# zju3dv/ENeRF

Hardware: AMD Instinct MI355X
Metric: rendered frames/sec @512x640 3-src-view (higher is better)
Workload: dtype f32

## Files before the change

### enerf_amd/csrc/common.h

```cpp
#pragma once

#ifdef ENERF_EMU
#include "hip_emu.h"
typedef emu_f32x4 f32x4;
#else
#include <hip/hip_runtime.h>
typedef float f32x4 __attribute__((ext_vector_type(4)));
#define ENERF_LAUNCH(kern, grid, block, shmem, stream, ...) \
    hipLaunchKernelGGL(kern, dim3(grid), dim3(block), (shmem), (stream), __VA_ARGS__)
#define ENERF_LAUNCH_SIMPLE ENERF_LAUNCH
#define ENERF_DYN_SMEM(type, name) \
    extern __shared__ __attribute__((aligned(16))) char enerf_dyn_smem_[]; \
    type* name = reinterpret_cast<type*>(enerf_dyn_smem_)
#define ENERF_OPAQUE_V(x) asm volatile("" : "+v"(x))
#endif
#ifdef ENERF_EMU
#define ENERF_OPAQUE_V(x) (void)(x)
#endif

#include <stdint.h>

namespace enerf {

__device__ __forceinline__ void wave_sync() {
// ... 170 lines not shown
}
__device__ __forceinline__ float group_max4(float v) {
#ifdef ENERF_EMU
    v = fmaxf(v, __shfl_xor(v, 16));
    v = fmaxf(v, __shfl_xor(v, 32));
    return v;
#else
    unsigned u = __float_as_uint(v);
    auto r = __builtin_amdgcn_permlane32_swap(u, u, false, false);
    v = fmaxf(__uint_as_float(r[0]), __uint_as_float(r[1]));
    u = __float_as_uint(v);
    r = __builtin_amdgcn_permlane16_swap(u, u, false, false);
    return fmaxf(__uint_as_float(r[0]), __uint_as_float(r[1]));
#endif
}

__device__ __forceinline__ unsigned xcd_contiguous(unsigned bid, unsigned nblk) {
    const unsigned q = nblk / 8, r = nblk % 8, xcd = bid % 8, k = bid / 8;
    return (xcd < r ? xcd * (q + 1) : r * (q + 1) + (xcd - r) * q) + k;
}
__host__ __device__ __forceinline__ long long cdivl(long long a, long long b) { return (a + b - 1) / b; }

struct Lerp1 {
    int i0, i1;
    float l0, l1;
};
__host__ __device__ __forceinline__ float ac_scale(int in, int out) {
    return out > 1 ? (float)(in - 1) / (float)(out - 1) : 0.f;
}
__host__ __device__ __forceinline__ Lerp1 ac_lerp(int dst, float scale, int in) {
    Lerp1 r;
    float src = scale * (float)dst;
    r.i0 = (int)src;
    if (r.i0 > in - 1) r.i0 = in - 1;
    r.i1 = r.i0 + (r.i0 < in - 1 ? 1 : 0);
    r.l1 = src - (float)r.i0;
    r.l0 = 1.f - r.l1;
    return r;
}
__host__ __device__ __forceinline__ float ac_blend(const Lerp1& y, const Lerp1& x, float v00, float v01, float v10,
                                                   float v11) {
    return y.l0 * (x.l0 * v00 + x.l1 * v01) + y.l1 * (x.l0 * v10 + x.l1 * v11);
}

__host__ __device__ __forceinline__ float gs_unnorm(float g, int size) { return ((g + 1.f) * 0.5f) * (float)(size - 1); }

struct Taps2 {
    int x0, x1, y0, y1;
    float w00, w01, w10, w11;
};
__device__ __forceinline__ int mul24(int a, int b) {
#ifdef ENERF_EMU
    return a * b;
#else
    return __mul24(a, b);
#endif
}

template <bool BORDER>
__host__ __device__ __forceinline__ Taps2 gs_taps2(float ix, float iy, int W, int H) {
    Taps2 t;
    if (BORDER) {
        ix = fminf((float)(W - 1), fmaxf(ix, 0.f));
        iy = fminf((float)(H - 1), fmaxf(iy, 0.f));
        const float fx = floorf(ix), fy = floorf(iy);
        t.x0 = (int)fx; t.y0 = (int)fy;
        t.x1 = t.x0 + 1 < W ? t.x0 + 1 : W - 1;
        t.y1 = t.y0 + 1 < H ? t.y0 + 1 : H - 1;
        const float tx1 = ix - fx, ty1 = iy - fy, tx0 = (fx + 1.f) - ix, ty0 = (fy + 1.f) - iy;
        t.w00 = tx0 * ty0; t.w01 = tx1 * ty0; t.w10 = tx0 * ty1; t.w11 = tx1 * ty1;
        return t;
    }
    bool finite = (ix > -1e8f) && (ix < 1e8f) && (iy > -1e8f) && (iy < 1e8f);
    if (!finite) { ix = -10.f; iy = -10.f; }
    float fx = floorf(ix), fy = floorf(iy);
    int x0 = (int)fx, y0 = (int)fy;
    int x1 = x0 + 1, y1 = y0 + 1;
    float tx1 = ix - fx, ty1 = iy - fy;
    float tx0 = (float)x1 - ix, ty0 = (float)y1 - iy;
    bool vx0 = x0 >= 0 && x0 < W, vx1 = x1 >= 0 && x1 < W;
    bool vy0 = y0 >= 0 && y0 < H, vy1 = y1 >= 0 && y1 < H;
    t.w00 = (vx0 && vy0) ? tx0 * ty0 : 0.f;
    t.w01 = (vx1 && vy0) ? tx1 * ty0 : 0.f;
    t.w10 = (vx0 && vy1) ? tx0 * ty1 : 0.f;
    t.w11 = (vx1 && vy1) ? tx1 * ty1 : 0.f;
    t.x0 = x0 < 0 ? 0 : (x0 > W - 1 ? W - 1 : x0);
    t.x1 = x1 < 0 ? 0 : (x1 > W - 1 ? W - 1 : x1);
    t.y0 = y0 < 0 ? 0 : (y0 > H - 1 ? H - 1 : y0);
    t.y1 = y1 < 0 ? 0 : (y1 > H - 1 ? H - 1 : y1);
    return t;
}

__device__ __forceinline__ float clamp_min(float v, float lo) { return v < lo ? lo : v; }

__device__ __forceinline__ void atomic_add_f32(float* p, float v) {
#ifdef ENERF_EMU
    atomicAdd(p, v);
#else
    unsafeAtomicAdd(p, v);
#endif
}

__device__ __forceinline__ void lds_add_f32(float* p, float v) {
#ifdef ENERF_EMU
    atomicAdd(p, v);
#else
    __builtin_amdgcn_ds_faddf((__attribute__((address_space(3))) float*)p, v, 0, 0, false);
#endif
}

#ifdef ENERF_EMU
__device__ __forceinline__ float fast_rcp(float x) { return 1.f / x; }
__device__ __forceinline__ float fast_sqrt(float x) { return sqrtf(x); }
__device__ __forceinline__ float fast_exp(float x) { return expf(x); }
#else
__device__ __forceinline__ float fast_rcp(float x) { return __builtin_amdgcn_rcpf(x); }
__device__ __forceinline__ float fast_sqrt(float x) { return __builtin_amdgcn_sqrtf(x); }
__device__ __forceinline__ float fast_exp(float x) { return __expf(x); }
#endif

__host__ __device__ __forceinline__ float linspace01(int k, int D) {
    if (D == 1) return 0.f;
    float step = 1.f / (float)(D - 1);
    return k < D / 2 ? step * (float)k : 1.f - step * (float)(D - 1 - k);
}

__host__ __device__ __forceinline__ bool inv4x4(const double* m, double* inv) {
    inv[0] = m[5] * m[10] * m[15] - m[5] * m[11] * m[14] - m[9] * m[6] * m[15] + m[9] * m[7] * m[14] + m[13] * m[6] * m[11] - m[13] * m[7] * m[10];
    inv[4] = -m[4] * m[10] * m[15] + m[4] * m[11] * m[14] + m[8] * m[6] * m[15] - m[8] * m[7] * m[14] - m[12] * m[6] * m[11] + m[12] * m[7] * m[10];
    inv[8] = m[4] * m[9] * m[15] - m[4] * m[11] * m[13] - m[8] * m[5] * m[15] + m[8] * m[7] * m[13] + m[12] * m[5] * m[11] - m[12] * m[7] * m[9];
    inv[12] = -m[4] * m[9] * m[14] + m[4] * m[10] * m[13] + m[8] * m[5] * m[14] - m[8] * m[6] * m[13] - m[12] * m[5] * m[10] + m[12] * m[6] * m[9];
    inv[1] = -m[1] * m[10] * m[15] + m[1] * m[11] * m[14] + m[9] * m[2] * m[15] - m[9] * m[3] * m[14] - m[13] * m[2] * m[11] + m[13] * m[3] * m[10];
    inv[5] = m[0] * m[10] * m[15] - m[0] * m[11] * m[14] - m[8] * m[2] * m[15] + m[8] * m[3] * m[14] + m[12] * m[2] * m[11] - m[12] * m[3] * m[10];
    inv[9] = -m[0] * m[9] * m[15] + m[0] * m[11] * m[13] + m[8] * m[1] * m[15] - m[8] * m[3] * m[13] - m[12] * m[1] * m[11] + m[12] * m[3] * m[9];
    inv[13] = m[0] * m[9] * m[14] - m[0] * m[10] * m[13] - m[8] * m[1] * m[14] + m[8] * m[2] * m[13] + m[12] * m[1] * m[10] - m[12] * m[2] * m[9];
    inv[2] = m[1] * m[6] * m[15] - m[1] * m[7] * m[14] - m[5] * m[2] * m[15] + m[5] * m[3] * m[14] + m[13] * m[2] * m[7] - m[13] * m[3] * m[6];
    inv[6] = -m[0] * m[6] * m[15] + m[0] * m[7] * m[14] + m[4] * m[2] * m[15] - m[4] * m[3] * m[14] - m[12] * m[2] * m[7] + m[12] * m[3] * m[6];
    inv[10] = m[0] * m[5] * m[15] - m[0] * m[7] * m[13] - m[4] * m[1] * m[15] + m[4] * m[3] * m[13] + m[12] * m[1] * m[7] - m[12] * m[3] * m[5];
    inv[14] = -m[0] * m[5] * m[14] + m[0] * m[6] * m[13] + m[4] * m[1] * m[14] - m[4] * m[2] * m[13] - m[12] * m[1] * m[6] + m[12] * m[2] * m[5];
    inv[3] = -m[1] * m[6] * m[11] + m[1] * m[7] * m[10] + m[5] * m[2] * m[11] - m[5] * m[3] * m[10] - m[9] * m[2] * m[7] + m[9] * m[3] * m[6];
    inv[7] = m[0] * m[6] * m[11] - m[0] * m[7] * m[10] - m[4] * m[2] * m[11] + m[4] * m[3] * m[10] + m[8] * m[2] * m[7] - m[8] * m[3] * m[6];
    inv[11] = -m[0] * m[5] * m[11] + m[0] * m[7] * m[9] + m[4] * m[1] * m[11] - m[4] * m[3] * m[9] - m[8] * m[1] * m[7] + m[8] * m[3] * m[5];
    inv[15] = m[0] * m[5] * m[10] - m[0] * m[6] * m[9] - m[4] * m[1] * m[10] + m[4] * m[2] * m[9] + m[8] * m[1] * m[6] - m[8] * m[2] * m[5];
    double det = m[0] * inv[0] + m[1] * inv[4] + m[2] * inv[8] + m[3] * inv[12];
    if (det == 0.0) return false;
    double r = 1.0 / det;
    for (int i = 0; i < 16; ++i) inv[i] *= r;
    return true;
}

struct RayBounds {
    float rn, rf, vn, vf;
};
__device__ __forceinline__ RayBounds ray_bounds(float ru, float rv, const float* __restrict__ pd,
                                                const float* __restrict__ ps, const float* __restrict__ n0,
                                                int h, int w, int Hr, int Wr, int depth_inv) {
    int u = (int)ru, v = (int)rv;
    u = u < 0 ? u + Wr : u;
    v = v < 0 ? v + Hr : v;
    u = u < 0 ? 0 : (u > Wr - 1 ? Wr - 1 : u);
    v = v < 0 ? 0 : (v > Hr - 1 ? Hr - 1 : v);
    const Lerp1 ly = ac_lerp(v, ac_scale(h, Hr), h), lx = ac_lerp(u, ac_scale(w, Wr), w);
    const int o00 = ly.i0 * w + lx.i0, o01 = ly.i0 * w + lx.i1, o10 = ly.i1 * w + lx.i0, o11 = ly.i1 * w + lx.i1;
    const float* n1 = n0 + h * w;
    float d, s, a0, a1;
    if ((h == Hr) && (w == Wr)) {
        d = pd[o00]; s = ps[o00]; a0 = n0[o00]; a1 = n1[o00];
    } else {
        d = ac_blend(ly, lx, pd[o00], pd[o01], pd[o10], pd[o11]);
        s = ac_blend(ly, lx, ps[o00], ps[o01], ps[o10], ps[o11]);
        a0 = ac_blend(ly, lx, n0[o00], n0[o01], n0[o10], n0[o11]);
        a1 = ac_blend(ly, lx, n1[o00], n1[o01], n1[o10], n1[o11]);
    }
    RayBounds r;
    if (depth_inv) {
        r.rn = d + s; if (r.rn > a0) r.rn = a0;
        r.rf = d - s; if (r.rf < a1) r.rf = a1;
    } else {
        r.rn = d - s; if (r.rn < a0) r.rn = a0;
        r.rf = d + s; if (r.rf > a1) r.rf = a1;
    }
    r.vn = a0; r.vf = a1;
    return r;
}

}
```

### enerf_amd/csrc/render.hip

```cpp
#include "nerf_layout.h"

#ifndef ENERF_RENDER_PREFETCH
#define ENERF_RENDER_PREFETCH 0
#endif

namespace enerf {

__host__ __device__ __forceinline__ int bx_image_floats(int F, int pieces = 3) { return F == 11 ? bx_layout().tiles * 256 * pieces : 0; }
long long nerf_packed_floats(int F) { return nerf_layout(F).total + bx_image_floats(F); }

__host__ __device__ __forceinline__ int slot_channel(int g, int r, int R, int F) {
    int c = g * R + r;
    return (r < R && c < F) ? c : -1;
}

__device__ __forceinline__ float bx_weight(const NerfRaw& w, int F, int e, int g, int j, int q) {
    const int R = (F + 3) / 4, CI = 88 + F + 4;
    const BxLayout B = bx_layout();
    const int half = q >> 2, r = q & 3;
    const int c = (r < R && g * R + r < F) ? g * R + r : -1;
    if (e < B.ga) return c >= 0 ? w.glob_w[(16 * e + j) * 3 * F + (1 + half) * F + c] : 0.f;
    if (e < B.fc) return (half == 0 && c >= 0) ? w.glob_w[(16 * (e - B.ga) + j) * 3 * F + c] : 0.f;
    if (e < B.lr0) return w.fc_w[j * 32 + 16 * half + 4 * g + r];
    if (e < B.c0p) {
        const int unit = 16 * (e - B.lr0) + j;
        if (half == 0) return r < 2 ? w.lr0_w[unit * 24 + 2 * g + r] : 0.f;
        return w.lr0_w[unit * 24 + 8 + 4 * g + r];
    }
    if (e < B.c0v) {
        const int pr = (e - B.c0p) >> 2, unit = 16 * ((e - B.c0p) & 3) + j;
        if (pr < 2) return w.col0_w[unit * CI + 16 * (2 * pr + half) + 4 * g + r];
        if (half == 0) return r < 2 ? w.col0_w[unit * CI + 64 + 2 * g + r] : 0.f;
        return w.col0_w[unit * CI + 72 + 4 * g + r];
    }
    if (half) return 0.f;
    const int unit = 16 * (e - B.c0v) + j;
    if (c >= 0) return w.col0_w[unit * CI + 88 + c];
    return r == R ? w.col0_w[unit * CI + 88 + F + g] : 0.f;
}
__device__ __forceinline__ unsigned bf16_bits_rne(float f) {
    unsigned u = __float_as_uint(f);
    return (u + 0x7fffu + ((u >> 16) & 1u)) >> 16;
}
__global__ __launch_bounds__(256) void k_nerf_pack(NerfRaw w, int F, int viewdir_agg, float* __restrict__ out) {
    const NerfLayout L = nerf_layout(F);
    int i = blockIdx.x * blockDim.x + threadIdx.x;
    if (i >= L.total + bx_image_floats(F)) return;
    if (i >= L.total) {
        const int idx = i - L.total, n_plane = bx_layout().tiles * 256;
        const int piece = idx / n_plane, k = idx - piece * n_plane;
        const int e = k >> 8, lane = (k >> 2) & 63, wq = k & 3;
        unsigned word = 0;
        for (int h = 0; h < 2; ++h) {
            float rem = bx_weight(w, F, e, lane >> 4, lane & 15, 2 * wq + h);
            unsigned bits = 0;
            for (int pc = 0; pc <= piece; ++pc) { bits = bf16_bits_rne(rem); rem -= __uint_as_float(bits << 16); }
            word |= (bits & 0xffffu) << (16 * h);
        }
        out[i] = __uint_as_float(word);
        return;
    }
    const int R = L.R;
    const int CI = 88 + F + 4;
    float v = 0.f;
    auto mfma_lane = [&](int rel, int& e, int& g, int& row) { e = rel >> 6; g = (rel & 63) >> 4; row = rel & 15; };
    int e, g, row;
    if (i >= L.col2) {
        int k = i - L.col2;
        if (k < 64) v = w.col2_w[k]; else if (k == 64) v = w.col2_b[0];
    } else if (i >= L.c0v) {
        mfma_lane(i - L.c0v, e, g, row);
        int ks = e >> 2, vt = e & 3, unit = 16 * vt + row;
        if (ks < R) { int c = slot_channel(g, ks, R, F); if (c >= 0) v = w.col0_w[unit * CI + 88 + c]; }
        else if (ks == R) v = w.col0_w[unit * CI + 88 + F + g];
    } else if (i >= L.c0b) {
        int k = i - L.c0b; if (k < 64) v = w.col0_b[k];
    } else if (i >= L.c0p) {
        mfma_lane(i - L.c0p, e, g, row);
        int ks = e >> 2, vt = e & 3, unit = 16 * vt + row;
        if (ks < 16) v = w.col0_w[unit * CI + 16 * (ks >> 2) + 4 * g + (ks & 3)];
        else if (ks < 18) v = w.col0_w[unit * CI + 64 + 2 * g + (ks - 16)];
        else if (ks < 22) v = w.col0_w[unit * CI + 72 + 4 * g + (ks - 18)];
    } else if (i >= L.sigma) {
        int k = i - L.sigma;
        if (k < 64) v = w.sigma_w[k]; else if (k == 64) v = w.sigma_b[0];
    } else if (i >= L.lr0b) {
        int k = i - L.lr0b; if (k < 64) v = w.lr0_b[k];
    } else if (i >= L.lr0) {
        mfma_lane(i - L.lr0, e, g, row);
        int ks = e >> 2, vt = e & 3, unit = 16 * vt + row;
        if (ks < 2) v = w.lr0_w[unit * 24 + 2 * g + ks];
        else if (ks < 6) v = w.lr0_w[unit * 24 + 8 + 4 * g + (ks - 2)];
    } else if (i >= L.fcb) {
        int k = i - L.fcb; if (k < 16) v = w.fc_b[k];
    } else if (i >= L.fc) {
        mfma_lane(i - L.fc, e, g, row);
        if (e < 8) v = w.fc_w[row * 32 + 16 * (e >> 2) + 4 * g + (e & 3)];
    } else if (i >= L.aggw) {
        int k = i - L.aggw;
        if (k < 32) v = w.aggw_w[k]; else if (k == 32) v = w.aggw_b[0];
    } else if (i >= L.globb) {
        int k = i - L.globb; if (k < 32) v = w.glob_b[k];
    } else if (i >= L.glob) {
        mfma_lane(i - L.glob, e, g, row);
        int u = e & 1, pr = e >> 1, part = pr / R, r = pr - part * R;
        int c = slot_channel(g, r, R, F);
        if (part < 3 && c >= 0) v = w.glob_w[(16 * u + row) * 3 * F + part * F + c];
    } else if (i >= L.viewb) {
        int k = i - L.viewb;
        int t = k >> 4, rr = k & 15;
        int c = slot_channel(rr >> 2, 4 * t + (rr & 3), R, F);
        if (t < L.TR && c >= 0 && viewdir_agg) v = w.view_b[c];
    } else {
        mfma_lane(i - L.view, e, g, row);
        int c = slot_channel(row >> 2, 4 * e + (row & 3), R, F);
        if (e < L.TR && c >= 0 && viewdir_agg) v = w.view_w[c * 4 + g];
    }
    out[i] = v;
}
void launch_nerf_pack(const NerfRaw& raw, int F, int viewdir_agg, float* packed, hipStream_t st) {
    int total = (int)nerf_packed_floats(F);
    ENERF_LAUNCH_SIMPLE(k_nerf_pack, cdiv(total, 256), 256, 0, st, raw, F, viewdir_agg, packed);
}

constexpr int kCamStride = 16;

template <int R> struct Stage { static constexpr int kTex = 4 * R, kStride = 4 * R + 8; };

template <int R, int S, int WAVES, int WPE, bool PFK = false, bool LEANK = false, int BX = 0>
__global__ __launch_bounds__(64 * WAVES)
#ifndef ENERF_EMU
__attribute__((amdgpu_waves_per_eu(WPE, WPE)))
#endif
void k_render_rays(RenderArgs a) {
    static_assert(BX == 0 || R == 3, "the bf16 image exists for F = 11 only");
    constexpr bool BX3 = BX != 0;
    constexpr int NP = BX == 6 ? 3 : 2;
    constexpr int TR = (R + 3) / 4;
    constexpr int TEX = Stage<R>::kTex, SST = Stage<R>::kStride;
    const NerfLayout LF = nerf_layout(a.F);
    const NerfLayout L = nerf_layout(a.F, BX3);
    constexpr int BXP = 25 * 256;
    constexpr int BXF = BX3 ? BXP * NP : 0;
    ENERF_DYN_SMEM(float, smem);
    float* wl = smem;
    const float* bx = smem + L.total;
    auto bxplane = [&](int q) { return bx + q * BXP; };
    float* cam = smem + L.total + BXF;
    float* tcen = cam + a.B * S * kCamStride;
    float* stage_all = tcen + ((a.B * 4 + 15) & ~15);

    {
        constexpr int MAXW4 = (BX3 ? BXF : (R == 3 ? 10560 : 14528)) / 4;
        constexpr int NWI = (MAXW4 + 64 * WAVES - 1) / (64 * WAVES);
        float4 wq[NWI];
        const int n4 = (BX3 ? BXF : L.total) / 4;
        const float* src = a.packed + (BX3 ? LF.total : 0);
        float* dst = BX3 ? smem + L.total : wl;
#pragma unroll
        for (int it = 0; it < NWI; ++it) {
            const int i = (int)threadIdx.x + it * 64 * WAVES;
            wq[it] = *reinterpret_cast<const float4*>(src + (i < n4 ? i : n4 - 1) * 4);
        }
#pragma unroll
        for (int it = 0; it < NWI; ++it) {
            const int i = (int)threadIdx.x + it * 64 * WAVES;
            if (i < n4) *reinterpret_cast<float4*>(dst + i * 4) = wq[it];
        }
        if (BX3) {
            const int so[9] = {LF.view, LF.viewb, LF.globb, LF.aggw, LF.fcb, LF.lr0b, LF.sigma, LF.c0b, LF.col2};
            const int dd[9] = {L.view, L.viewb, L.globb, L.aggw, L.fcb, L.lr0b, L.sigma, L.c0b, L.col2};
            const int nn[9] = {L.TR * 64, L.TR * 16, 32, 33, 16, 64, 65, 64, 65};
            for (int q = 0; q < 9; ++q)
                for (int i = threadIdx.x; i < nn[q]; i += blockDim.x) wl[dd[q] + i] = a.packed[so[q] + i];
        }
    }
    for (int i = threadIdx.x; i < a.B * (S + 1); i += blockDim.x) {
        int b = i / (S + 1), s = i - b * (S + 1);
        const float* E = (s < S) ? a.src_exts + ((long long)b * S + s) * 16 : a.tar_ext + (long long)b * 16;
        double m[16], inv[16];
        for (int k = 0; k < 16; ++k) m[k] = (double)E[k];
        bool ok = inv4x4(m, inv);
        float c0 = ok ? (float)inv[3] : NAN, c1 = ok ? (float)inv[7] : NAN, c2 = ok ? (float)inv[11] : NAN;
        if (s < S) {
            float* c = cam + ((long long)b * S + s) * kCamStride;
            const float* K = a.src_ixts + ((long long)b * S + s) * 9;
            for (int r = 0; r < 3; ++r) {
                double kr[3];
                for (int q = 0; q < 3; ++q) kr[q] = (double)K[r * 3 + q] * (r < 2 ? (double)a.render_scale : 1.0);
                for (int q = 0; q < 4; ++q) {
                    const double v = kr[0] * m[q] + kr[1] * m[4 + q] + kr[2] * m[8 + q];
                    if (q < 3) c[r * 3 + q] = (float)v; else c[9 + r] = (float)v;
                }
            }
            c[12] = c0; c[13] = c1; c[14] = c2; c[15] = 0.f;
        } else {
            tcen[b * 4 + 0] = c0; tcen[b * 4 + 1] = c1; tcen[b * 4 + 2] = c2; tcen[b * 4 + 3] = 0.f;
        }
    }
    __syncthreads();

    const int lane = threadIdx.x & 63, g = lane >> 4, j = lane & 15;
    const int wave_in_block = threadIdx.x >> 6;
    const long long nrays = a.ray_index != nullptr ? (long long)a.ray_count[0] : (long long)a.B * a.N;
    const long long ntiles = cdivl(nrays, 16);
    const bool scatter = a.ray_index != nullptr && a.scatter_rgb != 0;
    const int Ns = a.n_samples;
    const float* wlane = wl + lane;
#define A_VIEW(e) wlane[L.view + (e) * 64]
#define A_GLOB(e) wlane[L.glob + (e) * 64]
#define A_FC(e) wlane[L.fc + (e) * 64]
#define A_LR0(e) wlane[L.lr0 + (e) * 64]
#define A_C0P(e) wlane[L.c0p + (e) * 64]
#define A_C0V(e) wlane[L.c0v + (e) * 64]
    float* stage = stage_all + wave_in_block * ((PFK ? 2 : 1) * S * 16 * SST);
    const int sv = g < S ? g : S - 1;
    float* my_rec = stage + (sv * 16 + j) * SST;
    const float* rd_rec = stage + j * SST + g * R;
    const float* rd_dir = stage + j * SST + TEX + g;

    const long long nbands = gridDim.x < 8 ? gridDim.x : 8;
    const long long xcd_ = blockIdx.x % nbands, nb8 = ((long long)gridDim.x + nbands - 1 - xcd_) / nbands, bi_ = blockIdx.x / nbands;
    const long long t_hi = ntiles * (xcd_ + 1) / nbands;
#ifndef ENERF_RENDER_BALANCE_R9
#define ENERF_RENDER_BALANCE_R9 1
#endif
    const long long t_lo = ntiles * xcd_ / nbands, per_round = nb8 * WAVES, full = (t_hi - t_lo) / per_round;
    const long long rem = (t_hi - t_lo) - full * per_round, rb = rem / nb8, rx = rem - rb * nb8;
    const long long my_rem = rb + (bi_ < rx ? 1 : 0), my_rem_lo = bi_ * rb + (bi_ < rx ? bi_ : rx);
    constexpr bool kBal = R == 3 || ENERF_RENDER_BALANCE_R9;
    const long long n_it = kBal ? full + (wave_in_block < my_rem ? 1 : 0)
                                : full + (full * per_round + bi_ * WAVES + wave_in_block < t_hi - t_lo ? 1 : 0);
    for (long long it = 0; it < n_it; ++it) {
        const long long tile = (it < full || !kBal) ? t_lo + it * per_round + bi_ * WAVES + wave_in_block
                                                    : t_lo + full * per_round + my_rem_lo + wave_in_block;
        long long ray = tile * 16 + j;
        const bool rok = ray < nrays;
        const long long rc = rok ? ray : nrays - 1;
        const long long rr = a.ray_index != nullptr ? (long long)a.ray_index[rc] : rc;
        const int b = (int)(rr / a.N);
        float ox, oy, oz, dx, dy, dz, ru, rv, rn, rf, vn, vf;
        if (a.rays8 != nullptr) {
            const float* rp = a.rays8 + rr * 8;
            const float4 q0 = *reinterpret_cast<const float4*>(rp), q1 = *reinterpret_cast<const float4*>(rp + 4);
            ox = q0.x; oy = q0.y; oz = q0.z; dx = q0.w; dy = q1.x; dz = q1.y; ru = q1.z; rv = q1.w;
            const long long mo = (long long)b * a.map_h * a.map_w;
            const RayBounds rb = ray_bounds(ru, rv, a.depth_map + mo, a.std_map + mo, a.nf_map + 2 * mo, a.map_h, a.map_w,
                                            a.Hr, a.Wr, a.depth_inv);
            rn = rb.rn; rf = rb.rf; vn = rb.vn; vf = rb.vf;
        } else {
            const float* rp = a.rays12 + rr * 12;
            const float4 q0 = *reinterpret_cast<const float4*>(rp), q1 = *reinterpret_cast<const float4*>(rp + 4),
                         q2 = *reinterpret_cast<const float4*>(rp + 8);
            ox = q0.x; oy = q0.y; oz = q0.z; dx = q0.w; dy = q1.x; dz = q1.y; ru = q1.z; rv = q1.w;
            rn = q2.x; rf = q2.y; vn = q2.z; vf = q2.w;
        }
        const unsigned voff = (unsigned)b * (unsigned)(a.D * a.h * a.w * 8) + 2u * g;
        float wxy[4];
        int oxy[4];
        {
            const float gxv = (ru / (float)(a.Wr - 1)) * 2.f - 1.f, gyv = (rv / (float)(a.Hr - 1)) * 2.f - 1.f;
            float ix = gs_unnorm(gxv, a.w), iy = gs_unnorm(gyv, a.h);
            ix = fabsf(ix) < 1e8f ? ix : -10.f;
            iy = fabsf(iy) < 1e8f ? iy : -10.f;
            const float fx = floorf(ix), fy = floorf(iy);
            const int x0 = (int)fx, y0 = (int)fy;
            float wx[2] = {(fx + 1.f) - ix, ix - fx}, wy[2] = {(fy + 1.f) - iy, iy - fy};
            int xo[2], yo[2];
#pragma unroll
            for (int c = 0; c < 2; ++c) {
                const int xx = x0 + c, yy = y0 + c;
                wx[c] = (unsigned)xx < (unsigned)a.w ? wx[c] : 0.f;
                wy[c] = (unsigned)yy < (unsigned)a.h ? wy[c] : 0.f;
                xo[c] = min(max(xx, 0), a.w - 1);
                yo[c] = mul24(min(max(yy, 0), a.h - 1), a.w);
            }
#pragma unroll
            for (int c = 0; c < 4; ++c) { wxy[c] = wx[c & 1] * wy[c >> 1]; oxy[c] = yo[c >> 1] + xo[c & 1]; }
        }
        const float* cb = cam + ((long long)b * S + sv) * kCamStride;
        f32x4 cm0, cm1, cm2, cm3, tc4;
        if (!LEANK) { cm0 = lds4(cb); cm1 = lds4(cb + 4); cm2 = lds4(cb + 8); cm3 = lds4(cb + 12); tc4 = lds4(tcen + b * 4); }
        const unsigned toff = (unsigned)b * (unsigned)(S * a.Hr * a.Wr * TEX) + (unsigned)sv * (unsigned)(a.Hr * a.Wr * TEX);
        const float rcpW = fast_rcp((float)(a.Wr - 1)), rcpH = fast_rcp((float)(a.Hr - 1));

        float Tacc = 1.f;
        constexpr int NSM = (LEANK && R == 3) ? 2 : 8;
        float wk[NSM];
        float rgbacc[R];
#pragma unroll
        for (int r = 0; r < R; ++r) rgbacc[r] = 0.f;
#pragma unroll
        for (int k = 0; k < NSM; ++k) wk[k] = 0.f;

        struct GatherRegs {
            float2 vt[8];
            f32x4 tq[(R <= 3 ? 1 : 2)][4][(R <= 3 ? R : 3)];
            unsigned tp[4];
            float tw[4], wz[2];
            f32x4 dirc;
        };
        constexpr int QB = R <= 3 ? R : 3, NRND = R / QB, NBUF = NRND > 1 ? 2 : 1;
        static_assert(R % QB == 0, "texel chunk rounds");
        const char* const texb = reinterpret_cast<const char*>(a.tex);
        const char* const volb = reinterpret_cast<const char*>(a.vol);
        auto gather_issue = [&](int k, GatherRegs& G) {
            if (LEANK) { cm0 = lds4(cb); cm1 = lds4(cb + 4); cm2 = lds4(cb + 8); cm3 = lds4(cb + 12); tc4 = lds4(tcen + b * 4); }
            float tk = (Ns == 1) ? 0.5f : linspace01(k, Ns);
            float z = rn + (rf - rn) * tk;
            float zz = a.depth_inv ? fast_rcp(clamp_min(z, 1e-6f)) : z;
            float X = ox + dx * zz, Y = oy + dy * zz, Z = oz + dz * zz;
            float dn = a.depth_inv ? (vn - z) * fast_rcp(clamp_min(vn - vf, 1e-6f))
                                   : (z - vn) * fast_rcp(clamp_min(vf - vn, 1e-6f));
            const float px = X * cm0[0] + Y * cm0[1] + Z * cm0[2] + cm2[1];
            const float py = X * cm0[3] + Y * cm1[0] + Z * cm1[1] + cm2[2];
            const float pz = X * cm1[2] + Y * cm1[3] + Z * cm2[0] + cm2[3];
            const float rz = fast_rcp(clamp_min(pz, 1e-6f));
            const float gx = ((px * rz) * rcpW) * 2.f - 1.f, gy = ((py * rz) * rcpH) * 2.f - 1.f;
            const Taps2 t = gs_taps2<true>(gs_unnorm(gx, a.Wr), gs_unnorm(gy, a.Hr), a.Wr, a.Hr);
            const int r0 = mul24(t.y0, a.Wr), r1 = mul24(t.y1, a.Wr);
            G.tp[0] = (toff + (unsigned)mul24(r0 + t.x0, TEX)) * 4u; G.tp[1] = (toff + (unsigned)mul24(r0 + t.x1, TEX)) * 4u;
            G.tp[2] = (toff + (unsigned)mul24(r1 + t.x0, TEX)) * 4u; G.tp[3] = (toff + (unsigned)mul24(r1 + t.x1, TEX)) * 4u;
            G.tw[0] = t.w00; G.tw[1] = t.w01; G.tw[2] = t.w10; G.tw[3] = t.w11;
            float iz = gs_unnorm(dn * 2.f - 1.f, a.D);
            iz = fabsf(iz) < 1e8f ? iz : -10.f;
            const float fz = floorf(iz);
            const int z0 = (int)fz;
            G.wz[0] = (fz + 1.f) - iz; G.wz[1] = iz - fz;
            int zo[2];
#pragma unroll
            for (int c = 0; c < 2; ++c) {
                const int zc = z0 + c;
                G.wz[c] = (unsigned)zc < (unsigned)a.D ? G.wz[c] : 0.f;
                zo[c] = mul24(min(max(zc, 0), a.D - 1), a.h * a.w);
            }
            __builtin_amdgcn_sched_barrier(0);
#pragma unroll
            for (int c = 0; c < 8; ++c)
                G.vt[c] = *reinterpret_cast<const float2*>(volb + ((unsigned)(zo[c >> 2] + oxy[c & 3]) * 8u + voff) * 4u);
#pragma unroll
            for (int rd = 0; rd < NBUF; ++rd)
#pragma unroll
                for (int c = 0; c < 4; ++c)
#pragma unroll
                    for (int q = 0; q < QB; ++q) G.tq[rd][c][q] = lds4(reinterpret_cast<const float*>(texb + G.tp[c]) + 4 * (rd * QB + q));
            __builtin_amdgcn_sched_barrier(0);
            float tx = X - tc4[0], ty = Y - tc4[1], tz = Z - tc4[2];
            float sx = X - cm3[0], sy = Y - cm3[1], sz = Z - cm3[2];
            const float tir = fast_rcp(fast_sqrt(tx * tx + ty * ty + tz * tz) + 1e-6f);
            const float sir = fast_rcp(fast_sqrt(sx * sx + sy * sy + sz * sz) + 1e-6f);
            tx *= tir; ty *= tir; tz *= tir;
            sx *= sir; sy *= sir; sz *= sir;
            const float ex = tx - sx, ey = ty - sy, ez = tz - sz;
            const float eir = fast_rcp(fmaxf(fast_sqrt(ex * ex + ey * ey + ez * ez), 1e-6f));
            G.dirc = f32x4{ex * eir, ey * eir, ez * eir, tx * sx + ty * sy + tz * sz};
        };
        auto gather_finish = [&](GatherRegs& G, float* rec, float (&vox)[2]) {
            float vw[8];
#pragma unroll
            for (int c = 0; c < 8; ++c) vw[c] = wxy[c & 3] * G.wz[c >> 2];
            __builtin_amdgcn_sched_barrier(0);
            f32x4 blend[R];
#pragma unroll
            for (int rd = 0; rd < NRND; ++rd) {
#pragma unroll
                for (int q = 0; q < QB; ++q) {
                    f32x4 acc = G.tq[rd % NBUF][0][q] * G.tw[0];
                    acc += G.tq[rd % NBUF][1][q] * G.tw[1];
                    acc += G.tq[rd % NBUF][2][q] * G.tw[2];
                    acc += G.tq[rd % NBUF][3][q] * G.tw[3];
                    blend[rd * QB + q] = acc;
                }
                if (rd + NBUF < NRND) {
                    __builtin_amdgcn_sched_barrier(0);
#pragma unroll
                    for (int c = 0; c < 4; ++c)
#pragma unroll
                        for (int q = 0; q < QB; ++q) G.tq[rd % NBUF][c][q] = lds4(reinterpret_cast<const float*>(texb + G.tp[c]) + 4 * ((rd + NBUF) * QB + q));
                    __builtin_amdgcn_sched_barrier(0);
                }
            }
            if (g < S) {
#pragma unroll
                for (int q = 0; q < R; ++q) *reinterpret_cast<f32x4*>(rec + 4 * q) = blend[q];
                *reinterpret_cast<f32x4*>(rec + TEX) = G.dirc;
            }
            vox[0] = 0.f; vox[1] = 0.f;
#pragma unroll
            for (int c = 0; c < 8; ++c) {
                vox[0] += G.vt[c].x * vw[c];
                vox[1] += G.vt[c].y * vw[c];
            }
        };
        constexpr bool PF = PFK;
        constexpr int RECBUF = S * 16 * SST;
        GatherRegs GR;
        float vox_next[2] = {0.f, 0.f};
        if (PF) {
            gather_issue(0, GR);
            gather_finish(GR, my_rec, vox_next);
        }
#pragma unroll 1
        for (int k = 0; k < Ns; ++k) {
            asm volatile("" ::: "memory");
            float vox[2];
            const int rb = PF ? (k & 1) * RECBUF : 0;
            if (!PF) {
                gather_issue(k, GR);
                gather_finish(GR, my_rec, vox);
            } else {
                vox[0] = vox_next[0]; vox[1] = vox_next[1];
            }
            wave_sync();
            float x[S][R], dsel[S];
#pragma unroll
            for (int s = 0; s < S; ++s) {
#pragma unroll
                for (int r = 0; r < R; ++r) x[s][r] = rd_rec[rb + s * 16 * SST + r];
                dsel[s] = rd_dir[rb + s * 16 * SST];
            }
            wave_sync();
            const bool more = PF && k + 1 < Ns;
            if (more) gather_issue(k + 1, GR);

            float av[S][R];
            {
                float aview[TR];
#pragma unroll
                for (int t = 0; t < TR; ++t) aview[t] = A_VIEW(t);
                f32x4 vb[TR];
#pragma unroll
                for (int t = 0; t < TR; ++t) vb[t] = lds4(wl + L.viewb + t * 16 + 4 * g);
#pragma unroll
// ... 79 lines not shown
                for (int s = 0; s < S; ++s) { aw[s] = fast_exp(aw[s] - m); se += aw[s]; }
                se = fast_rcp(se);
#pragma unroll
                for (int s = 0; s < S; ++s) aw[s] *= se;
            }
            f32x4 G[2];
#pragma unroll
            for (int u = 0; u < 2; ++u) {
                G[u] = gf[0][u] * aw[0];
#pragma unroll
                for (int s = 1; s < S; ++s) G[u] += gf[s][u] * aw[s];
            }
            f32x4 aggv[1] = {lds4(wl + L.fcb + 4 * g)};
            if constexpr (BX3) {
                const BxLayout BL = bx_layout();
                bfx8 gp[NP];
                bx_split<NP>(G[0], G[1], gp);
                bx_mma_n<NP, 1>(bxplane, BL.fc, lane, gp, aggv);
            } else {
                float afc[8];
#pragma unroll
                for (int e = 0; e < 8; ++e) afc[e] = A_FC(e);
                __builtin_amdgcn_sched_barrier(0);
#pragma unroll
                for (int e = 0; e < 8; ++e) aggv[0] = ENERF_MFMA(afc[e], G[e >> 2][e & 3], aggv[0]);
            }
            const f32x4 agg = relu4(aggv[0]);

            if (more) gather_finish(GR, my_rec + ((k + 1) & 1) * RECBUF, vox_next);

            f32x4 hid[4];
#pragma unroll
            for (int v = 0; v < 4; ++v) hid[v] = lds4(wl + L.lr0b + v * 16 + 4 * g);
            bfx8 vap[NP];
            if constexpr (BX3) {
                const BxLayout BL = bx_layout();
                bx_split<NP>(f32x4{vox[0], vox[1], 0.f, 0.f}, agg, vap);
                bx_mma_n<NP, 4>(bxplane, BL.lr0, lane, vap, hid);
            } else
            mfma_chain<6, 4>(hid, [&](int e) { return A_LR0(e); }, [&](int ks) { return ks < 2 ? vox[ks < 2 ? ks : 0] : agg[ks >= 2 ? ks - 2 : 0]; });
            float sig = 0.f;
#pragma unroll
            for (int v = 0; v < 4; ++v) {
                hid[v] = relu4(hid[v]);
                sig = dot4(hid[v], lds4(wl + L.sigma + v * 16 + 4 * g), sig);
            }
            sig = group_sum(sig) + wl[L.sigma + 64];
            sig = sig > 20.f ? sig : log1pf(expf(sig));

            f32x4 P2[4];
#pragma unroll
            for (int v = 0; v < 4; ++v) P2[v] = lds4(wl + L.c0b + v * 16 + 4 * g);
            if constexpr (BX3) {
                const BxLayout BL = bx_layout();
#pragma unroll
                for (int pr = 0; pr < 2; ++pr) {
                    bfx8 hp[NP];
                    bx_split<NP>(hid[2 * pr], hid[2 * pr + 1], hp);
                    bx_mma_n<NP, 4>(bxplane, BL.c0p + 4 * pr, lane, hp, P2);
                }
                bx_mma_n<NP, 4>(bxplane, BL.c0p + 8, lane, vap, P2);
            } else
            mfma_chain<22, 4>(P2, [&](int e) { return A_C0P(e); },
                              [&](int ks) { return ks < 16 ? hid[(ks < 16 ? ks : 0) >> 2][ks & 3]
                                                           : (ks < 18 ? vox[ks < 18 ? ks - 16 : 0] : agg[ks >= 18 ? ks - 18 : 0]); });
            float cl[S];
            const float c2b = wl[L.col2 + 64];
            if constexpr (BX3) {
                const BxLayout BL = bx_layout();
                const f32x4 zero4 = {0.f, 0.f, 0.f, 0.f};
                f32x4 c2w[4];
#pragma unroll
                for (int v = 0; v < 4; ++v) c2w[v] = lds4(wl + L.col2 + v * 16 + 4 * g);
#pragma unroll
                for (int s = 0; s < S; ++s) {
                    bfx8 xp[NP];
                    bx_split<NP>(f32x4{x[s][0], x[s][1], x[s][2], dsel[s]}, zero4, xp);
                    f32x4 cc[4] = {P2[0], P2[1], P2[2], P2[3]};
                    bx_mma_n<NP, 4>(bxplane, BL.c0v, lane, xp, cc);
                    float part = 0.f;
#pragma unroll
                    for (int v = 0; v < 4; ++v) part = dot4(relu4(cc[v]), c2w[v], part);
                    cl[s] = relu1(group_sum(part) + c2b);
                }
            } else
            {
                float acv[(R + 1) * 4];
#pragma unroll
                for (int e = 0; e < (R + 1) * 4; ++e) acv[e] = A_C0V(e);
                f32x4 c2w[4];
#pragma unroll
                for (int v = 0; v < 4; ++v) c2w[v] = lds4(wl + L.col2 + v * 16 + 4 * g);
                __builtin_amdgcn_sched_barrier(0);
#pragma unroll
                for (int s = 0; s < S; ++s) {
                    f32x4 cc[4];
#pragma unroll
                    for (int v = 0; v < 4; ++v) cc[v] = P2[v];
#pragma unroll
                    for (int ks = 0; ks <= R; ++ks) {
                        float bop = ks < R ? x[s][ks < R ? ks : 0] : dsel[s];
#pragma unroll
                        for (int v = 0; v < 4; ++v) cc[v] = ENERF_MFMA(acv[ks * 4 + v], bop, cc[v]);
                    }
                    float part = 0.f;
#pragma unroll
                    for (int v = 0; v < 4; ++v) part = dot4(relu4(cc[v]), c2w[v], part);
                    cl[s] = relu1(group_sum(part) + c2b);
                }
            }
            {
                float m = cl[0];
#pragma unroll
                for (int s = 1; s < S; ++s) m = fmaxf(m, cl[s]);
                float se = 0.f;
#pragma unroll
                for (int s = 0; s < S; ++s) { cl[s] = fast_exp(cl[s] - m); se += cl[s]; }
                se = fast_rcp(se);
#pragma unroll
                for (int s = 0; s < S; ++s) cl[s] *= se;
            }

            float alpha = 1.f - fast_exp(-sig);
            float wgt = alpha * Tacc;
            Tacc *= (1.f - alpha + 1e-10f);
#pragma unroll
            for (int r = 0; r < R; ++r) {
                float col = x[0][r] * cl[0];
#pragma unroll
                for (int s = 1; s < S; ++s) col += x[s][r] * cl[s];
                rgbacc[r] += wgt * col;
            }
#pragma unroll
            for (int kk = 0; kk < NSM; ++kk)
                if (kk == k) wk[kk] = wgt;
        }

        float m = wk[0];
#pragma unroll
        for (int k = 1; k < NSM; ++k) if (k < Ns) m = fmaxf(m, wk[k]);
        float se = 0.f;
#pragma unroll
        for (int k = 0; k < NSM; ++k) if (k < Ns) { wk[k] = fast_exp(wk[k] - m); se += wk[k]; }
        se = fast_rcp(se);
        float depth = 0.f, accw = 0.f;
#pragma unroll
        for (int k = 0; k < NSM; ++k)
            if (k < Ns) {
                wk[k] *= se;
                float tk = (Ns == 1) ? 0.5f : linspace01(k, Ns);
                depth += wk[k] * (rn + (rf - rn) * tk);
                accw += wk[k];
            }
        if (rok) {
#pragma unroll
            for (int r = 0; r < R; ++r) {
                int c = g * R + r - (a.F - 3);
                if (c >= 0 && c < 3) {
                    float v = rgbacc[r];
                    if (a.white_bkgd) v += 1.f - accw;
                    if (!scatter) a.rgb[ray * 3 + c] = v;
                    else if (nrays > 1) a.rgb[rr * 3 + c] = v;
                }
            }
            if (g == 0) {
                a.depth[ray] = depth;
#pragma unroll
                for (int k = 0; k < NSM; ++k) if (k < Ns) a.weights[ray * Ns + k] = wk[k];
            }
        }
    }
}

template <int R, int WAVES, int OCC, bool PFK = false, bool LEANK = false, int BX3 = 0>
static int dispatch_s(const RenderArgs& a, unsigned grid, size_t shmem, hipStream_t st) {
    constexpr int WPE = (WAVES * OCC + 3) / 4;
    switch (a.S) {
        case 2: ENERF_LAUNCH((k_render_rays<R, 2, WAVES, WPE, PFK, LEANK, BX3>), grid, 64 * WAVES, shmem, st, a); return 0;
        case 3: ENERF_LAUNCH((k_render_rays<R, 3, WAVES, WPE, PFK, LEANK, BX3>), grid, 64 * WAVES, shmem, st, a); return 0;
        case 4: ENERF_LAUNCH((k_render_rays<R, 4, WAVES, WPE, PFK, LEANK, BX3>), grid, 64 * WAVES, shmem, st, a); return 0;
        default: return -3;
    }
}
template <int R, int WAVES>
static size_t render_shmem(const RenderArgs& a, int record_buffers = 1, int bx = 0) {
    return ((size_t)nerf_layout(a.F, bx != 0).total + (size_t)(bx ? bx_image_floats(a.F, bx == 6 ? 3 : 2) : 0) + (size_t)a.B * a.S * kCamStride + (size_t)((a.B * 4 + 15) & ~15) +
            (size_t)WAVES * record_buffers * a.S * 16 * Stage<R>::kStride) * sizeof(float);
}
int launch_render_rays(const RenderArgs& a, hipStream_t st) {
    if (a.n_samples < 1 || a.n_samples > 8) return -1;
    const int R = (a.F + 3) / 4;
    if ((long long)a.B * a.S * a.Hr * a.Wr * 4 * R >= (1LL << 30) || (long long)a.B * a.D * a.h * a.w * 8 >= (1LL << 30) ||
        (long long)a.Hr * a.Wr >= (1LL << 23) || (long long)a.h * a.w >= (1LL << 23) || a.D >= (1 << 23))
        return -5;
    const long long ntiles = cdivl((long long)a.B * a.N, 16);
    const int cus = device_cu_count();
    auto grid_for = [&](int waves, int occ) {
        const long long blocks = cdivl(ntiles, waves);
        long long resident = (long long)cus * occ;
        if (a.max_blocks > 0 && a.max_blocks < resident) resident = a.max_blocks;
        return (unsigned)(blocks < resident ? blocks : resident);
    };
#ifndef ENERF_R9_LEAN
#define ENERF_R9_LEAN 1
#endif
#ifndef ENERF_RENDER_LEAN12
#define ENERF_RENDER_LEAN12 1
#endif
#ifndef ENERF_RENDER_WAVES
#define ENERF_RENDER_WAVES 4
#endif
#ifndef ENERF_RENDER_OCC
#define ENERF_RENDER_OCC 2
#endif
    if (nerf_layout(a.F).total > (R == 3 ? 10560 : 14528)) return -6;
    if (R == 3 && a.n_samples <= 2 && ENERF_RENDER_LEAN12) {
        const int prec = a.options != nullptr ? a.options->render_precision : 0;
        const int bx = prec == 2 ? 3 : (prec == 3 ? 6 : 0);
        const size_t shmem = render_shmem<3, 12>(a, 1, bx);
        if (shmem <= 160 * 1024) {
            const unsigned grid = grid_for(12, 1);
            if (grid == 0) return 0;
            if (bx == 6) return dispatch_s<3, 12, 1, false, true, 6>(a, grid, shmem, st);
            if (bx == 3) return dispatch_s<3, 12, 1, false, true, 3>(a, grid, shmem, st);
            return dispatch_s<3, 12, 1, false, true>(a, grid, shmem, st);
        }
    }
    if (R == 3) {
        const size_t shmem = render_shmem<3, ENERF_RENDER_WAVES>(a);
        if (shmem > 160 * 1024 / ENERF_RENDER_OCC) return -2;
        const unsigned grid = grid_for(ENERF_RENDER_WAVES, ENERF_RENDER_OCC);
        if (grid == 0) return 0;
        const size_t shmem_pf = render_shmem<3, ENERF_RENDER_WAVES>(a, 2);
        if (ENERF_RENDER_PREFETCH != 0 && a.n_samples > 1 && shmem_pf <= 160 * 1024 / ENERF_RENDER_OCC)
            return dispatch_s<3, ENERF_RENDER_WAVES, ENERF_RENDER_OCC, true>(a, grid, shmem_pf, st);
        return dispatch_s<3, ENERF_RENDER_WAVES, ENERF_RENDER_OCC>(a, grid, shmem, st);
    }
    if (R == 9) {
        const size_t shmem = render_shmem<9, 8>(a);
        if (shmem > 160 * 1024) return -2;
        unsigned grid = grid_for(8, 1);
        if (0 && ENERF_RENDER_BALANCE_R9 && ntiles > 0) {
            const long long t = cdivl(ntiles, 4LL * cus), tight = cdivl(ntiles, 4 * t);
            if (tight < (long long)grid) grid = (unsigned)tight;
        }
        if (grid == 0) return 0;
        return dispatch_s<9, 8, 1, false, ENERF_R9_LEAN != 0>(a, grid, shmem, st);
    }
    return -4;
}

}
```

Baseline: 1321.

## Batch per-ray setup across several tiles per wave, staged in LDS

```diff
diff --git a/enerf_amd/csrc/common.h b/enerf_amd/csrc/common.h
--- a/enerf_amd/csrc/common.h
+++ b/enerf_amd/csrc/common.h
@@ -346,9 +346,8 @@
 struct RayBounds {
     float rn, rf, vn, vf;
 };
-__device__ __forceinline__ RayBounds ray_bounds(float ru, float rv, const float* __restrict__ pd,
-                                                const float* __restrict__ ps, const float* __restrict__ n0,
-                                                int h, int w, int Hr, int Wr, int depth_inv) {
+template <class LD>
+__device__ __forceinline__ RayBounds ray_bounds_ld(float ru, float rv, int h, int w, int Hr, int Wr, int depth_inv, LD&& ld) {
     int u = (int)ru, v = (int)rv;
     u = u < 0 ? u + Wr : u;
     v = v < 0 ? v + Hr : v;
@@ -356,15 +355,14 @@
     v = v < 0 ? 0 : (v > Hr - 1 ? Hr - 1 : v);
     const Lerp1 ly = ac_lerp(v, ac_scale(h, Hr), h), lx = ac_lerp(u, ac_scale(w, Wr), w);
     const int o00 = ly.i0 * w + lx.i0, o01 = ly.i0 * w + lx.i1, o10 = ly.i1 * w + lx.i0, o11 = ly.i1 * w + lx.i1;
-    const float* n1 = n0 + h * w;
     float d, s, a0, a1;
     if ((h == Hr) && (w == Wr)) {
-        d = pd[o00]; s = ps[o00]; a0 = n0[o00]; a1 = n1[o00];
+        d = ld(0, o00); s = ld(1, o00); a0 = ld(2, o00); a1 = ld(3, o00);
     } else {
-        d = ac_blend(ly, lx, pd[o00], pd[o01], pd[o10], pd[o11]);
-        s = ac_blend(ly, lx, ps[o00], ps[o01], ps[o10], ps[o11]);
-        a0 = ac_blend(ly, lx, n0[o00], n0[o01], n0[o10], n0[o11]);
-        a1 = ac_blend(ly, lx, n1[o00], n1[o01], n1[o10], n1[o11]);
+        d = ac_blend(ly, lx, ld(0, o00), ld(0, o01), ld(0, o10), ld(0, o11));
+        s = ac_blend(ly, lx, ld(1, o00), ld(1, o01), ld(1, o10), ld(1, o11));
+        a0 = ac_blend(ly, lx, ld(2, o00), ld(2, o01), ld(2, o10), ld(2, o11));
+        a1 = ac_blend(ly, lx, ld(3, o00), ld(3, o01), ld(3, o10), ld(3, o11));
     }
     RayBounds r;
     if (depth_inv) {
@@ -377,5 +375,12 @@
     r.vn = a0; r.vf = a1;
     return r;
 }
-
-}
+__device__ __forceinline__ RayBounds ray_bounds(float ru, float rv, const float* __restrict__ pd,
+                                                const float* __restrict__ ps, const float* __restrict__ n0,
+                                                int h, int w, int Hr, int Wr, int depth_inv) {
+    const float* n1 = n0 + h * w;
+    return ray_bounds_ld(ru, rv, h, w, Hr, Wr, depth_inv,
+                         [&](int m, int o) { return m == 0 ? pd[o] : (m == 1 ? ps[o] : (m == 2 ? n0[o] : n1[o])); });
+}
+
+}
diff --git a/enerf_amd/csrc/render.hip b/enerf_amd/csrc/render.hip
--- a/enerf_amd/csrc/render.hip
+++ b/enerf_amd/csrc/render.hip
@@ -127,13 +127,16 @@
 
 template <int R> struct Stage { static constexpr int kTex = 4 * R, kStride = 4 * R + 8; };
 
+constexpr int kSetupStride = 20;
+
 template <int R, int S, int WAVES, int WPE, bool PFK = false, bool LEANK = false, int BX = 0>
 __global__ __launch_bounds__(64 * WAVES)
 #ifndef ENERF_EMU
 __attribute__((amdgpu_waves_per_eu(WPE, WPE)))
 #endif
-void k_render_rays(RenderArgs a) {
+void k_render_rays(RenderArgs a, int tb, int idx32) {
     static_assert(BX == 0 || R == 3, "the bf16 image exists for F = 11 only");
+    constexpr bool TBK = LEANK && R == 3 && !PFK;
     constexpr bool BX3 = BX != 0;
     constexpr int NP = BX == 6 ? 3 : 2;
     constexpr int TR = (R + 3) / 4;
@@ -201,7 +204,7 @@
     __syncthreads();
 
     const int lane = threadIdx.x & 63, g = lane >> 4, j = lane & 15;
-    const int wave_in_block = threadIdx.x >> 6;
+    const int wave_in_block = __builtin_amdgcn_readfirstlane((int)(threadIdx.x >> 6));
     const long long nrays = a.ray_index != nullptr ? (long long)a.ray_count[0] : (long long)a.B * a.N;
     const long long ntiles = cdivl(nrays, 16);
     const bool scatter = a.ray_index != nullptr && a.scatter_rgb != 0;
@@ -214,6 +217,8 @@
 #define A_C0P(e) wlane[L.c0p + (e) * 64]
 #define A_C0V(e) wlane[L.c0v + (e) * 64]
     float* stage = stage_all + wave_in_block * ((PFK ? 2 : 1) * S * 16 * SST);
+    static_assert(S * SST >= kSetupStride, "one tile's setup records fit the wave's (view, point) records");
+    float* setup = (TBK && tb > 1) ? stage_all + WAVES * ((PFK ? 2 : 1) * S * 16 * SST) + wave_in_block * (tb * 16 * kSetupStride) : stage;
     const int sv = g < S ? g : S - 1;
     float* my_rec = stage + (sv * 16 + j) * SST;
     const float* rd_rec = stage + j * SST + g * R;
@@ -225,39 +230,55 @@
 #ifndef ENERF_RENDER_BALANCE_R9
 #define ENERF_RENDER_BALANCE_R9 1
 #endif
-    const long long t_lo = ntiles * xcd_ / nbands, per_round = nb8 * WAVES, full = (t_hi - t_lo) / per_round;
-    const long long rem = (t_hi - t_lo) - full * per_round, rb = rem / nb8, rx = rem - rb * nb8;
-    const long long my_rem = rb + (bi_ < rx ? 1 : 0), my_rem_lo = bi_ * rb + (bi_ < rx ? bi_ : rx);
+    const long long t_lo_ = ntiles * xcd_ / nbands, per_round = nb8 * WAVES, full_ = (t_hi - t_lo_) / per_round;
+    const long long rem = (t_hi - t_lo_) - full_ * per_round, rb = rem / nb8, rx = rem - rb * nb8;
+    const long long my_rem = rb + (bi_ < rx ? 1 : 0), my_rem_lo_ = bi_ * rb + (bi_ < rx ? bi_ : rx);
     constexpr bool kBal = R == 3 || ENERF_RENDER_BALANCE_R9;
-    const long long n_it = kBal ? full + (wave_in_block < my_rem ? 1 : 0)
-                                : full + (full * per_round + bi_ * WAVES + wave_in_block < t_hi - t_lo ? 1 : 0);
-    for (long long it = 0; it < n_it; ++it) {
-        const long long tile = (it < full || !kBal) ? t_lo + it * per_round + bi_ * WAVES + wave_in_block
-                                                    : t_lo + full * per_round + my_rem_lo + wave_in_block;
-        long long ray = tile * 16 + j;
-        const bool rok = ray < nrays;
-        const long long rc = rok ? ray : nrays - 1;
-        const long long rr = a.ray_index != nullptr ? (long long)a.ray_index[rc] : rc;
-        const int b = (int)(rr / a.N);
+    auto uniform = [](long long v) {
+        return (long long)(((unsigned long long)(unsigned)__builtin_amdgcn_readfirstlane((int)(v >> 32)) << 32) | (unsigned)__builtin_amdgcn_readfirstlane((int)v));
+    };
+    const long long t_lo = uniform(t_lo_), my_rem_lo = uniform(my_rem_lo_);
+    const int full = __builtin_amdgcn_readfirstlane((int)full_);
+    const int n_it = __builtin_amdgcn_readfirstlane(kBal ? full + (wave_in_block < my_rem ? 1 : 0)
+                                                         : full + (full * per_round + bi_ * WAVES + wave_in_block < t_hi - t_lo ? 1 : 0));
+    const int t_lo32 = (int)t_lo, per_round32 = (int)per_round, wv32 = (int)(bi_ * WAVES + wave_in_block),
+              rem_tile32 = (int)(t_lo + full * per_round + my_rem_lo + wave_in_block);
+    auto tile_of = [&](int i, auto tag) {
+        if constexpr (sizeof(tag) == 4) return (i < full || !kBal) ? t_lo32 + i * per_round32 + wv32 : rem_tile32;
+        else return (i < full || !kBal) ? t_lo + i * per_round + bi_ * WAVES + wave_in_block
+                                        : t_lo + full * per_round + my_rem_lo + wave_in_block;
+    };
+    auto ldg = [&](auto tag, const void* base, auto off) {
+        using T = decltype(tag);
+        if constexpr (sizeof(off) == 4) return *reinterpret_cast<const T*>(reinterpret_cast<const char*>(base) + (unsigned)off);
+        else return *reinterpret_cast<const T*>(reinterpret_cast<const char*>(base) + off);
+    };
+    struct RaySetup { f32x4 q0, q1, q2, wxy; int oxy[4]; };
+    auto prepare = [&](auto tile) {
+        using IT = decltype(tile);
+        const IT ray = tile * 16 + j, nr = (IT)nrays;
+        const IT rc = ray < nr ? ray : nr - 1;
+        const IT rr = a.ray_index != nullptr ? (IT)ldg(int{}, a.ray_index, rc * 4) : rc;
+        int b = 0;
+        if (a.B != 1) {
+            if constexpr (sizeof(IT) == 4) b = (int)((unsigned)rr / (unsigned)a.N); else b = (int)(rr / a.N);
+        }
         float ox, oy, oz, dx, dy, dz, ru, rv, rn, rf, vn, vf;
         if (a.rays8 != nullptr) {
-            const float* rp = a.rays8 + rr * 8;
-            const float4 q0 = *reinterpret_cast<const float4*>(rp), q1 = *reinterpret_cast<const float4*>(rp + 4);
-            ox = q0.x; oy = q0.y; oz = q0.z; dx = q0.w; dy = q1.x; dz = q1.y; ru = q1.z; rv = q1.w;
-            const long long mo = (long long)b * a.map_h * a.map_w;
-            const RayBounds rb = ray_bounds(ru, rv, a.depth_map + mo, a.std_map + mo, a.nf_map + 2 * mo, a.map_h, a.map_w,
-                                            a.Hr, a.Wr, a.depth_inv);
+            const f32x4 q0 = ldg(f32x4{}, a.rays8, rr * 32), q1 = ldg(f32x4{}, a.rays8, rr * 32 + 16);
+            ox = q0[0]; oy = q0[1]; oz = q0[2]; dx = q0[3]; dy = q1[0]; dz = q1[1]; ru = q1[2]; rv = q1[3];
+            const IT hw = (IT)a.map_h * a.map_w, mo = (IT)b * hw;
+            const RayBounds rb = ray_bounds_ld(ru, rv, a.map_h, a.map_w, a.Hr, a.Wr, a.depth_inv, [&](int m, int o) {
+                return m == 0 ? ldg(float{}, a.depth_map, (mo + o) * 4)
+                              : (m == 1 ? ldg(float{}, a.std_map, (mo + o) * 4) : ldg(float{}, a.nf_map, (2 * mo + (m == 3 ? hw : 0) + o) * 4));
+            });
             rn = rb.rn; rf = rb.rf; vn = rb.vn; vf = rb.vf;
         } else {
-            const float* rp = a.rays12 + rr * 12;
-            const float4 q0 = *reinterpret_cast<const float4*>(rp), q1 = *reinterpret_cast<const float4*>(rp + 4),
-                         q2 = *reinterpret_cast<const float4*>(rp + 8);
-            ox = q0.x; oy = q0.y; oz = q0.z; dx = q0.w; dy = q1.x; dz = q1.y; ru = q1.z; rv = q1.w;
-            rn = q2.x; rf = q2.y; vn = q2.z; vf = q2.w;
-        }
-        const unsigned voff = (unsigned)b * (unsigned)(a.D * a.h * a.w * 8) + 2u * g;
-        float wxy[4];
-        int oxy[4];
+            const f32x4 q0 = ldg(f32x4{}, a.rays12, rr * 48), q1 = ldg(f32x4{}, a.rays12, rr * 48 + 16), q2 = ldg(f32x4{}, a.rays12, rr * 48 + 32);
+            ox = q0[0]; oy = q0[1]; oz = q0[2]; dx = q0[3]; dy = q1[0]; dz = q1[1]; ru = q1[2]; rv = q1[3];
+            rn = q2[0]; rf = q2[1]; vn = q2[2]; vf = q2[3];
+        }
+        RaySetup P;
         {
             const float gxv = (ru / (float)(a.Wr - 1)) * 2.f - 1.f, gyv = (rv / (float)(a.Hr - 1)) * 2.f - 1.f;
             float ix = gs_unnorm(gxv, a.w), iy = gs_unnorm(gyv, a.h);
@@ -276,9 +297,49 @@
                 yo[c] = mul24(min(max(yy, 0), a.h - 1), a.w);
             }
 #pragma unroll
-            for (int c = 0; c < 4; ++c) { wxy[c] = wx[c & 1] * wy[c >> 1]; oxy[c] = yo[c >> 1] + xo[c & 1]; }
-        }
-        const float* cb = cam + ((long long)b * S + sv) * kCamStride;
+            for (int c = 0; c < 4; ++c) { P.wxy[c] = wx[c & 1] * wy[c >> 1]; P.oxy[c] = yo[c >> 1] + xo[c & 1]; }
+        }
+        P.q0 = f32x4{ox, oy, oz, dx};
+        P.q1 = f32x4{dy, dz, __int_as_float(b), __int_as_float((int)rr)};
+        P.q2 = f32x4{rn, rf, vn, vf};
+        return P;
+    };
+    int slot = 0;
+    for (int it = 0; it < n_it; ++it) {
+        const long long tile = tile_of(it, 0LL);
+        RaySetup P;
+        if constexpr (TBK) {
+            if (slot == 0) {
+                const int left = n_it - it;
+                const bool mine = g < (left < tb ? left : tb);
+                const RaySetup W = idx32 ? prepare(tile_of(mine ? it + g : it, 0)) : prepare(tile_of(mine ? it + g : it, 0LL));
+                if (mine) {
+                    float* rec = setup + mul24(lane, kSetupStride);
+                    *reinterpret_cast<f32x4*>(rec) = W.q0; *reinterpret_cast<f32x4*>(rec + 4) = W.q1;
+                    *reinterpret_cast<f32x4*>(rec + 8) = W.q2; *reinterpret_cast<f32x4*>(rec + 12) = W.wxy;
+                    *reinterpret_cast<f32x4*>(rec + 16) = f32x4{__int_as_float(W.oxy[0]), __int_as_float(W.oxy[1]), __int_as_float(W.oxy[2]), __int_as_float(W.oxy[3])};
+                }
+            }
+            wave_sync();
+            const float* rec = setup + mul24(slot * 16 + j, kSetupStride);
+            P.q0 = lds4(rec); P.q1 = lds4(rec + 4); P.q2 = lds4(rec + 8); P.wxy = lds4(rec + 12);
+            const f32x4 o4 = lds4(rec + 16);
+#pragma unroll
+            for (int c = 0; c < 4; ++c) P.oxy[c] = __float_as_int(o4[c]);
+            wave_sync();
+            slot = slot + 1 == tb ? 0 : slot + 1;
+        } else {
+            P = prepare(tile);
+        }
+        const float ox = P.q0[0], oy = P.q0[1], oz = P.q0[2], dx = P.q0[3], dy = P.q1[0], dz = P.q1[1];
+        const float rn = P.q2[0], rf = P.q2[1], vn = P.q2[2], vf = P.q2[3];
+        const int b = __float_as_int(P.q1[2]);
+        float wxy[4];
+        int oxy[4];
+#pragma unroll
+        for (int c = 0; c < 4; ++c) { wxy[c] = P.wxy[c]; oxy[c] = P.oxy[c]; }
+        const unsigned voff = (unsigned)b * (unsigned)(a.D * a.h * a.w * 8) + 2u * g;
+        const float* cb = cam + (b * S + sv) * kCamStride;
         f32x4 cm0, cm1, cm2, cm3, tc4;
         if (!LEANK) { cm0 = lds4(cb); cm1 = lds4(cb + 4); cm2 = lds4(cb + 8); cm3 = lds4(cb + 12); tc4 = lds4(tcen + b * 4); }
         const unsigned toff = (unsigned)b * (unsigned)(S * a.Hr * a.Wr * TEX) + (unsigned)sv * (unsigned)(a.Hr * a.Wr * TEX);
@@ -664,43 +725,53 @@
                 depth += wk[k] * (rn + (rf - rn) * tk);
                 accw += wk[k];
             }
-        if (rok) {
+        auto store = [&](auto ray, auto rr) {
+            using IT = decltype(ray);
+            auto stg = [&](float* base, IT elem, float v) {
+                if constexpr (sizeof(IT) == 4) *reinterpret_cast<float*>(reinterpret_cast<char*>(base) + (unsigned)elem * 4u) = v;
+                else base[elem] = v;
+            };
+            if (ray >= (IT)nrays) return;
 #pragma unroll
             for (int r = 0; r < R; ++r) {
                 int c = g * R + r - (a.F - 3);
                 if (c >= 0 && c < 3) {
                     float v = rgbacc[r];
                     if (a.white_bkgd) v += 1.f - accw;
-                    if (!scatter) a.rgb[ray * 3 + c] = v;
-                    else if (nrays > 1) a.rgb[rr * 3 + c] = v;
+                    if (!scatter) stg(a.rgb, ray * 3 + c, v);
+                    else if (nrays > 1) stg(a.rgb, rr * 3 + c, v);
                 }
             }
             if (g == 0) {
-                a.depth[ray] = depth;
-#pragma unroll
-                for (int k = 0; k < NSM; ++k) if (k < Ns) a.weights[ray * Ns + k] = wk[k];
-            }
-        }
+                stg(a.depth, ray, depth);
+#pragma unroll
+                for (int k = 0; k < NSM; ++k) if (k < Ns) stg(a.weights, ray * Ns + k, wk[k]);
+            }
+        };
+        const int rr32 = __float_as_int(P.q1[3]);
+        if (TBK && idx32) store((int)tile * 16 + j, rr32); else store(tile * 16 + j, (long long)rr32);
     }
 }
 
 template <int R, int WAVES, int OCC, bool PFK = false, bool LEANK = false, int BX3 = 0>
-static int dispatch_s(const RenderArgs& a, unsigned grid, size_t shmem, hipStream_t st) {
+static int dispatch_s(const RenderArgs& a, unsigned grid, size_t shmem, hipStream_t st, int tb = 0) {
     constexpr int WPE = (WAVES * OCC + 3) / 4;
+    const int idx32 = (long long)a.B * a.N * 12 < (1LL << 29) && (a.rays8 == nullptr || (long long)a.B * a.map_h * a.map_w * 2 < (1LL << 29));
     switch (a.S) {
-        case 2: ENERF_LAUNCH((k_render_rays<R, 2, WAVES, WPE, PFK, LEANK, BX3>), grid, 64 * WAVES, shmem, st, a); return 0;
-        case 3: ENERF_LAUNCH((k_render_rays<R, 3, WAVES, WPE, PFK, LEANK, BX3>), grid, 64 * WAVES, shmem, st, a); return 0;
-        case 4: ENERF_LAUNCH((k_render_rays<R, 4, WAVES, WPE, PFK, LEANK, BX3>), grid, 64 * WAVES, shmem, st, a); return 0;
+        case 2: ENERF_LAUNCH((k_render_rays<R, 2, WAVES, WPE, PFK, LEANK, BX3>), grid, 64 * WAVES, shmem, st, a, tb, idx32); return 0;
+        case 3: ENERF_LAUNCH((k_render_rays<R, 3, WAVES, WPE, PFK, LEANK, BX3>), grid, 64 * WAVES, shmem, st, a, tb, idx32); return 0;
+        case 4: ENERF_LAUNCH((k_render_rays<R, 4, WAVES, WPE, PFK, LEANK, BX3>), grid, 64 * WAVES, shmem, st, a, tb, idx32); return 0;
         default: return -3;
     }
 }
 template <int R, int WAVES>
-static size_t render_shmem(const RenderArgs& a, int record_buffers = 1, int bx = 0) {
+static size_t render_shmem(const RenderArgs& a, int record_buffers = 1, int bx = 0, int tb = 0) {
     return ((size_t)nerf_layout(a.F, bx != 0).total + (size_t)(bx ? bx_image_floats(a.F, bx == 6 ? 3 : 2) : 0) + (size_t)a.B * a.S * kCamStride + (size_t)((a.B * 4 + 15) & ~15) +
-            (size_t)WAVES * record_buffers * a.S * 16 * Stage<R>::kStride) * sizeof(float);
+            (size_t)WAVES * record_buffers * a.S * 16 * Stage<R>::kStride + (size_t)(tb > 1 ? WAVES * tb * 16 * kSetupStride : 0)) * sizeof(float);
 }
 int launch_render_rays(const RenderArgs& a, hipStream_t st) {
     if (a.n_samples < 1 || a.n_samples > 8) return -1;
+    if ((long long)a.B * a.N >= (1LL << 35)) return -5;
     const int R = (a.F + 3) / 4;
     if ((long long)a.B * a.S * a.Hr * a.Wr * 4 * R >= (1LL << 30) || (long long)a.B * a.D * a.h * a.w * 8 >= (1LL << 30) ||
         (long long)a.Hr * a.Wr >= (1LL << 23) || (long long)a.h * a.w >= (1LL << 23) || a.D >= (1 << 23))
@@ -729,13 +800,15 @@
     if (R == 3 && a.n_samples <= 2 && ENERF_RENDER_LEAN12) {
         const int prec = a.options != nullptr ? a.options->render_precision : 0;
         const int bx = prec == 2 ? 3 : (prec == 3 ? 6 : 0);
-        const size_t shmem = render_shmem<3, 12>(a, 1, bx);
+        int tb = 4;
+        while (tb > 1 && render_shmem<3, 12>(a, 1, bx, tb) > 160 * 1024) tb >>= 1;
+        const size_t shmem = render_shmem<3, 12>(a, 1, bx, tb);
         if (shmem <= 160 * 1024) {
             const unsigned grid = grid_for(12, 1);
             if (grid == 0) return 0;
-            if (bx == 6) return dispatch_s<3, 12, 1, false, true, 6>(a, grid, shmem, st);
-            if (bx == 3) return dispatch_s<3, 12, 1, false, true, 3>(a, grid, shmem, st);
-            return dispatch_s<3, 12, 1, false, true>(a, grid, shmem, st);
+            if (bx == 6) return dispatch_s<3, 12, 1, false, true, 6>(a, grid, shmem, st, tb);
+            if (bx == 3) return dispatch_s<3, 12, 1, false, true, 3>(a, grid, shmem, st, tb);
+            return dispatch_s<3, 12, 1, false, true>(a, grid, shmem, st, tb);
         }
     }
     if (R == 3) {
```

Result: no change. 1326 (median of 3 runs) (+0.4%).
